# Ericonaldo/ILSwiss

Measured on AMD Instinct MI355X. Metric: env-steps/s + SAC grad-steps/s, Hopper-v2 4096 envs, higher is better.
Workload: dtype f32

## Files before the change

ilswiss_amd/csrc/host_common.h:

```cpp
#pragma once
#include <hip/hip_runtime.h>
#include <hip/hip_ext.h>

#include <cstdarg>
#include <cstdio>
#include <cstring>
#include <deque>
#include <string>
#include <utility>
#include <vector>

#include "../../include/ilsx.h"
#include "kernels.h"

void ilsx_set_err(const char* fmt, ...);

#define ILSX_FAIL(code, ...)   \
  do {                         \
    ilsx_set_err(__VA_ARGS__); \
    return (code);             \
  } while (0)

#define HIPCHK(expr)                                                                              \
  do {                                                                                            \
// ... 63 lines not shown
  std::vector<std::pair<void**, size_t>> items;
  size_t bytes = 0;
  template <class T> void add(T** p, size_t count) {
    bytes = (bytes + 255) & ~(size_t)255;
    items.push_back({(void**)p, bytes});
    bytes += count * sizeof(T);
  }
  int commit(ilsx_ctx* c, void** base) {
    int rc = ctx_alloc(c, bytes ? bytes : 256, base, true);
    if (rc != ILSX_OK) return rc;
    for (auto& it : items) *it.first = (char*)*base + it.second;
    return ILSX_OK;
  }
};
int ctx_free(ilsx_ctx* c, void* p);
int ctx_stage(ilsx_ctx* c, size_t bytes, void** out);

struct NetLayout {
  ilsx_mlp_cfg cfg;
  int KP = 0, NO = 0;
  int off_W[ILSX_MAX_HID], off_Wb[ILSX_MAX_HID], off_b[ILSX_MAX_HID], ld[ILSX_MAX_HID];
  int off_Wh = 0, off_bh = 0;
  size_t n_int = 0;
  size_t n_flat = 0;
  int hl[ILSX_MAX_HID] = {0, 0, 0};
  int out_of(int l) const { return hl[l] > 0 ? hl[l] : cfg.hidden; }
  int in_of(int l) const { return l == 0 ? cfg.in_dim : out_of(l - 1); }
};
int net_layout_build(const ilsx_mlp_cfg& cfg, NetLayout* L);
void net_flat_to_internal(const NetLayout& L, const float* flat, float* internal);
void net_internal_to_flat(const NetLayout& L, const float* internal, float* flat);
NetView net_view(const NetLayout& L, float* base);

struct ilsx_net {
  ilsx_ctx* ctx = nullptr;
  NetLayout lay;
  float* base = nullptr;
  bool owns = true;
  float* ws_out = nullptr;
  int ws_rows = 0;
  bool noise_policy = false;
  float noise = 0.f, noise_clip = 0.f, max_act = 1.f;
  bool out_linear = false;
  bool categorical = false;
};
int launch_categorical_act(ilsx_ctx* ctx, const float* z, int rows, int n, int deterministic, unsigned long long step, float* act, float* logp);

int net_upload_flat(ilsx_ctx* ctx, const NetLayout& L, float* dev_base, const float* src, size_t n, int src_is_device);
int net_download_flat(ilsx_ctx* ctx, const NetLayout& L, const float* dev_base, float* dst, size_t n, int dst_is_device);

int launch_fwd(ilsx_ctx* ctx, const FwdArgs& A, int H, int act, int KP, int cs = 1);
int launch_bwd_dx(ilsx_ctx* ctx, const BwdArgs& A, int H, int act, int cs = 1);
int launch_policy_finish(ilsx_ctx* ctx, const PolicyFinishArgs& P);
bool phase_fits(ilsx_ctx* ctx, int rows, int H, int cs, int ntasks);
struct PhaseConst {
  int slot = -1, device = 0;
  bool tried = false, valid_a = false, valid_c = false;
  unsigned long long key_a = 0, key_c = 0;
  PhaseAArgs a; PhaseCArgs c;
};
int phase_const_alloc(int device);
void phase_const_prepare(ilsx_ctx* ctx, PhaseConst* ct);
void phase_const_free(int device, int slot);
int launch_phase_a(ilsx_ctx* ctx, const PhaseAArgs& P, int H, int act, int KPmax, int cs, PhaseConst* ct = nullptr, unsigned long long key = 0, bool upload_only = false);
int launch_phase_c(ilsx_ctx* ctx, const PhaseCArgs& P, int H, int act, int KPmax, int cs, PhaseConst* ct = nullptr, unsigned long long key = 0, bool upload_only = false);
int device_cus(ilsx_ctx* ctx);
int grp_const_alloc(int device, bool fwd, int n, int* base);
void grp_const_free(int device, bool fwd, int base);
int grp_const_upload(ilsx_ctx* ctx, bool fwd, int base, const void* host_records, size_t count);
struct ilsx_sac;
int sac_staged_batch(ilsx_sac* s, int B, float** obs, float** act, float** rew, float** done, float** nobs);
int sac_step_staged(ilsx_sac* s, ilsx_sac_stats* stats);
int sac_dims(const ilsx_sac* s, int* o, int* a);
int sac_window_begin(ilsx_sac* s, int B);
int sac_window_step(ilsx_sac* s);
int sac_window_end(ilsx_sac* s, bool teardown = false);
#define ILSX_RETRY_WINDOW (-1000)
int sac_snapshot_take(ilsx_sac* s);
int sac_snapshot_restore(ilsx_sac* s);
bool sac_window_may_use_phase(ilsx_sac* s, int B);
int mlp2_split_factor(int n_hidden, int H);
int launch_bwd_dw(ilsx_ctx* ctx, const DwArgs& table, int rows, const AdamFuse* fuse = nullptr);
int dw_table_add(DwArgs* T, const float* A, int lda, int NA, const float* Bm, int ldb, int NB, float* dW, float* dWb, int ldw,
                 float* db, int mode, int rows = 0, int bias_rows = 0);
int launch_adam(ilsx_ctx* ctx, const AdamArgs& A);
int build_dw_jobs(const NetLayout& L, float* gbase, const float* xsave, float* const* hsave,
                  float* const* dsave, const float* dhead, DwArgs* table);

struct ilsx_replay {
  ilsx_ctx* ctx = nullptr;
  int64_t cap = 0;
  int o = 0, a = 0, rec = 0;
  float* data = nullptr;
  DevReplayState* dstate = nullptr;
  bool dstate_stale = false;
  uint64_t seed = 0;
  uint32_t rng_stream = 0;
  unsigned long long sample_ctr = 0;
  int64_t top = 0, size = 0, cur_start = 0;
  std::deque<std::pair<int64_t, int64_t>> trajs;
  std::vector<uint8_t> start_flag;
};
int replay_flush_state(ilsx_replay* rb);
int replay_advance_device_rows(ilsx_replay* rb, int n);
int replay_insert_paths(ilsx_replay* rb, const float* stage, int stage_len, const int* envs, const int* lens, const uint8_t* last_terminal,
                        int n_paths);
int replay_launch_sample(ilsx_replay* rb, int B, const int64_t* idx, const DevScalars* scal,
// ... 3 lines not shown
```

ilswiss_amd/csrc/ilsx_core.hip:

```cpp
#include <algorithm>
#include <cmath>
#include <cstdlib>
#include <random>

#define ILSX_KERNEL_IMPL 1
#include <mutex>
#include "host_common.h"

static thread_local std::string g_err = "";

void ilsx_set_err(const char* fmt, ...) {
  char buf[1024];
  va_list ap;
  va_start(ap, fmt);
  vsnprintf(buf, sizeof buf, fmt, ap);
  va_end(ap);
  g_err = buf;
}

static int kernels_init_once();
extern "C" int ilsx_abi_version(void) { return ILSX_ABI_VERSION; }
extern "C" const char* ilsx_last_error(void) { return g_err.c_str(); }

int ctx_alloc(ilsx_ctx* c, size_t bytes, void** out, bool zero) {
// ... 455 lines not shown
      if (act == ILSX_ACT_RELU) { if (gg == 2) L0_CALL(ACT_RELU, 2); else if (gg == 1) L0_CALL(ACT_RELU, 1); else L0_CALL(ACT_RELU, 0); }
      else { if (gg == 2) L0_CALL(ACT_TANH, 2); else if (gg == 1) L0_CALL(ACT_TANH, 1); else L0_CALL(ACT_TANH, 0); }
#undef L0_CALL
    } else if (H == 256 && cs == 4) {
#define FWD_GRP_CALL(HH, AA, CC) do { if (A.tasks && A.ctab && A.late) ILSX_LAUNCH(ps, (k_mlp2_fwd_split<HH, AA, CC, 3>), grid, block, lds, ctx->stream, A); \
        else if (A.tasks && A.ctab) ILSX_LAUNCH(ps, (k_mlp2_fwd_split<HH, AA, CC, 2>), grid, block, lds, ctx->stream, A); \
        else if (A.tasks) ILSX_LAUNCH(ps, (k_mlp2_fwd_split<HH, AA, CC, 1>), grid, block, lds, ctx->stream, A); \
        else ILSX_LAUNCH(ps, (k_mlp2_fwd_split<HH, AA, CC, 0>), grid, block, lds, ctx->stream, A); } while (0)
      if (act == ILSX_ACT_RELU) FWD_GRP_CALL(256, ACT_RELU, 4); else FWD_GRP_CALL(256, ACT_TANH, 4);
    } else if (H == 128 && cs == 2) {
      if (act == ILSX_ACT_RELU) FWD_GRP_CALL(128, ACT_RELU, 2); else FWD_GRP_CALL(128, ACT_TANH, 2);
#undef FWD_GRP_CALL
    } else {
      ILSX_FAIL(ILSX_ERR_UNSUPPORTED, "no column-split forward kernel for H=%d cs=%d", H, cs);
    }
    HIPCHK(hipGetLastError());
    return ILSX_OK;
  }
  const size_t lds = fwd_lds_bytes(H, KPmax);
  if (lds > 160 * 1024) ILSX_FAIL(ILSX_ERR_UNSUPPORTED, "forward tile needs %zu B of LDS (> 160 KiB)", lds);
  dim3 grid((A.rows + 15) / 16, A.ntasks), block(4 * H);
#define CALL_FWD(HH, AA) ILSX_LAUNCH(ps, (k_mlp_fwd<HH, AA>), grid, block, lds, ctx->stream, A)
  DISPATCH_H_ACT(H, act, CALL_FWD);
#undef CALL_FWD
  HIPCHK(hipGetLastError());
  return ILSX_OK;
}

int device_cus(ilsx_ctx* ctx) {
  static int n_cu = 0;
  if (!n_cu) {
    hipDeviceProp_t pr;
    n_cu = hipGetDeviceProperties(&pr, ctx->device) == hipSuccess ? pr.multiProcessorCount : 1;
  }
  return n_cu;
}
static size_t phase_lds_bytes(int H, int KP, int cs) { return std::max(fwd_split_lds_bytes(H, KP, cs), bwd_split_lds_bytes(H, cs)); }
void phase_wgs_per_cu(int H, int cs, int* occ_a, int* occ_c) {
  static int oa[2] = {-1, -1}, oc[2] = {-1, -1};
  const int i = H == 256 ? 0 : 1;
  if (oa[i] < 0) {
    int a = 0, c = 0;
    const size_t lds = phase_lds_bytes(H, 32, cs);
    hipError_t e1, e2;
    if (H == 256) { e1 = hipOccupancyMaxActiveBlocksPerMultiprocessor(&a, (const void*)k_sac_phase_a<256, ACT_RELU, 4>, 4 * H / cs, lds);
                    e2 = hipOccupancyMaxActiveBlocksPerMultiprocessor(&c, (const void*)k_sac_phase_c<256, ACT_RELU, 4>, 4 * H / cs, lds); }
    else { e1 = hipOccupancyMaxActiveBlocksPerMultiprocessor(&a, (const void*)k_sac_phase_a<128, ACT_RELU, 2>, 4 * H / cs, lds);
           e2 = hipOccupancyMaxActiveBlocksPerMultiprocessor(&c, (const void*)k_sac_phase_c<128, ACT_RELU, 2>, 4 * H / cs, lds); }
    oa[i] = e1 == hipSuccess ? std::max(a, 1) : 1;
    oc[i] = e2 == hipSuccess ? std::max(c, 1) : 1;
  }
  *occ_a = oa[i]; *occ_c = oc[i];
}
bool phase_fits(ilsx_ctx* ctx, int rows, int H, int cs, int ntasks) {
  const int n_cu = device_cus(ctx);
  if (!((H == 256 && cs == 4) || (H == 128 && cs == 2))) return false;
  const int tiles = (rows + 15) / 16, work = tiles * ntasks * cs;
  int occ_a = 1, occ_c = 1;
  phase_wgs_per_cu(H, cs, &occ_a, &occ_c);
  return tiles <= PHASE_MAX_TILES && work <= n_cu && work + 1 <= occ_a * n_cu && tiles * 3 * cs <= occ_c * n_cu;
}

static std::vector<bool> g_phase_slots[16];
static std::mutex g_phase_slots_mu;
int phase_const_alloc(int device) {
  static const bool off = []() { const char* e = getenv("ILSX_PHASE_CT"); return e && atoi(e) == 0; }();
  if (off || device < 0 || device >= 16) return -1;
  std::lock_guard<std::mutex> lock(g_phase_slots_mu);
  auto& u = g_phase_slots[device];
  if (u.empty()) u.assign(PHASE_CONST_SLOTS, false);
  for (int i = 0; i < PHASE_CONST_SLOTS; ++i) if (!u[i]) { u[i] = true; return i; }
  return -1;
}
void phase_const_free(int device, int slot) {
  if (device < 0 || device >= 16 || slot < 0 || slot >= PHASE_CONST_SLOTS) return;
  std::lock_guard<std::mutex> lock(g_phase_slots_mu);
  if (!g_phase_slots[device].empty()) g_phase_slots[device][slot] = false;
}
void phase_const_prepare(ilsx_ctx* ctx, PhaseConst* ct) {
  if (!ct || ct->tried) return;
  ct->tried = true;
  ct->device = ctx->device;
  ct->slot = phase_const_alloc(ctx->device);
  if (ct->slot >= 0) ctx->phase_slots.push_back(ct->slot);
}
template <class Blk>
static bool phase_const_ready(ilsx_ctx* ctx, PhaseConst* ct, const Blk& blk, unsigned long long key, Blk& held, bool& valid, unsigned long long& held_key,
                              const void* symbol) {
  phase_const_prepare(ctx, ct);
  if (!ct || ct->slot < 0 || blk.dbg || !key) return false;
  if (valid && held_key == key) return true;
  hipStreamCaptureStatus cap = hipStreamCaptureStatusNone;
  if (hipStreamIsCapturing(ctx->stream, &cap) != hipSuccess || cap != hipStreamCaptureStatusNone) return false;
  if (hipStreamSynchronize(ctx->stream) != hipSuccess) return false;
  valid = false;
  memcpy(&held, &blk, sizeof blk);
  if (hipMemcpyToSymbolAsync(symbol, &held, sizeof blk, (size_t)ct->slot * sizeof blk, hipMemcpyHostToDevice, ctx->stream) != hipSuccess ||
      hipStreamSynchronize(ctx->stream) != hipSuccess) { (void)hipGetLastError(); return false; }
  valid = true; held_key = key;
  return true;
}

int launch_phase_a(ilsx_ctx* ctx, const PhaseAArgs& P0, int H, int act, int KPmax, int cs, PhaseConst* ct, unsigned long long key, bool upload_only) {
  PhaseAArgs P = P0;
  P.f1.xs = P.f2.xs = P.b1.xs = 0; P.f1.rt = P.f2.rt = 1;
  P.f1.dbg = P.f2.dbg = nullptr; P.b1.dbg = nullptr;
  P.dbg = upload_only ? nullptr : ctx->dbg_next();
  if (P.b1.ga_parts < 1) P.b1.ga_parts = 1;
  const int tiles = (P.f1.rows + 15) / 16;
  dim3 grid((tiles + 7) & ~7, 5, cs), block(4 * H / cs);
  const size_t lds = phase_lds_bytes(H, KPmax, cs);
  const bool use_ct = ct && phase_const_ready(ctx, ct, P, key, ct->a, ct->valid_a, ct->key_a, HIP_SYMBOL(g_phase_a_tab));
  if (upload_only) return ILSX_OK;
  const int slot = use_ct ? ct->slot : 0;
  static const bool trace = getenv("ILSX_PHASE_CT_TRACE") != nullptr;
  if (trace) { hipStreamCaptureStatus cap = hipStreamCaptureStatusNone; hipStreamIsCapturing(ctx->stream, &cap);
               fprintf(stderr, "launch_phase_a: %s, slot %d, capturing %d\n", use_ct ? "constant table" : "kernel arguments", ct ? ct->slot : -9, (int)cap); }
  ProfScope ps(ctx, ILSX_K_SAC_PHASE_A);
#define PHASE_A(HH, AA, CC) do { if (use_ct) ILSX_LAUNCH(ps, (k_sac_phase_a<HH, AA, CC, true>), grid, block, lds, ctx->stream, P, slot); \
                                 else ILSX_LAUNCH(ps, (k_sac_phase_a<HH, AA, CC>), grid, block, lds, ctx->stream, P, slot); } while (0)
  if (H == 256 && act == ILSX_ACT_RELU) PHASE_A(256, ACT_RELU, 4);
  else if (H == 256) PHASE_A(256, ACT_TANH, 4);
  else if (act == ILSX_ACT_RELU) PHASE_A(128, ACT_RELU, 2);
  else PHASE_A(128, ACT_TANH, 2);
#undef PHASE_A
  HIPCHK(hipGetLastError());
  return ILSX_OK;
}

int launch_phase_c(ilsx_ctx* ctx, const PhaseCArgs& P0, int H, int act, int KPmax, int cs, PhaseConst* ct, unsigned long long key, bool upload_only) {
  PhaseCArgs P = P0;
  P.f3.xs = P.b2.xs = P.b3.xs = 0; P.f3.rt = 1;
  P.f3.dbg = nullptr; P.b2.dbg = P.b3.dbg = nullptr;
  P.dbg = upload_only ? nullptr : ctx->dbg_next();
  if (P.b2.ga_parts < 1) P.b2.ga_parts = 1;
  if (P.b3.ga_parts < 1) P.b3.ga_parts = 1;
  const int tiles = (P.f3.rows + 15) / 16;
  dim3 grid((tiles + 7) & ~7, 4, cs), block(4 * H / cs);
  const size_t lds = phase_lds_bytes(H, KPmax, cs);
  const bool use_ct = ct && phase_const_ready(ctx, ct, P, key, ct->c, ct->valid_c, ct->key_c, HIP_SYMBOL(g_phase_c_tab));
  if (upload_only) return ILSX_OK;
  const int slot = use_ct ? ct->slot : 0;
  ProfScope ps(ctx, ILSX_K_SAC_PHASE_C);
#define PHASE_C(HH, AA, CC) do { if (use_ct) ILSX_LAUNCH(ps, (k_sac_phase_c<HH, AA, CC, true>), grid, block, lds, ctx->stream, P, slot); \
                                 else ILSX_LAUNCH(ps, (k_sac_phase_c<HH, AA, CC>), grid, block, lds, ctx->stream, P, slot); } while (0)
  if (H == 256 && act == ILSX_ACT_RELU) PHASE_C(256, ACT_RELU, 4);
  else if (H == 256) PHASE_C(256, ACT_TANH, 4);
  else if (act == ILSX_ACT_RELU) PHASE_C(128, ACT_RELU, 2);
  else PHASE_C(128, ACT_TANH, 2);
#undef PHASE_C
  HIPCHK(hipGetLastError());
  return ILSX_OK;
}

int launch_bwd_dx(ilsx_ctx* ctx, const BwdArgs& A0, int H, int act, int cs) {
  if (A0.rows <= 0) return ILSX_OK;
  BwdArgs A = A0;
  A.dbg = ctx->dbg_next();
  if (A.ga_parts < 1) A.ga_parts = 1;
  ProfScope ps(ctx, ILSX_K_MLP_BWD_DX);
  if (cs > 1 && A.tasks && A.mt > 1) {
    if (!(H == 256 && cs == 4) || (A.mt != 2 && A.mt != 4)) ILSX_FAIL(ILSX_ERR_UNSUPPORTED, "macro-tile backward: H=%d cs=%d mt=%d", H, cs, A.mt);
    A.xs = 0; A.ctab = 0;
// ... 384 lines not shown
```

ilswiss_amd/csrc/ilsx_sac.hip:

```cpp
#include <cmath>
#include <cstdlib>

#include <algorithm>
#include "host_common.h"

enum { W_PI = 0, W_Q1 = 1, W_Q2 = 2, W_TQ1 = 3, W_TQ2 = 4 };

struct SacWs {
  float *s, *a, *r, *d, *s2, *eps1, *eps2;
  float *a2, *logp2, *q1, *q2, *tq1, *tq2;
  float *xq[2], *hq[2][ILSX_MAX_HID], *dq[2][ILSX_MAX_HID], *dhq[2];
  float *raw, *an, *logp, *epss, *q1n, *q2n, *ga[2];
  float *xp, *hp[ILSX_MAX_HID], *dp[ILSX_MAX_HID], *dhp;
  float* ppart;
  float* ppart2;
};

struct StatsArgs {
  PartVal q1, q2, tq1, tq2, q1n, q2n;
  const float *logp2, *r, *d, *logp, *raw;
  int B, a;
  float gamma, reward_scale, w_mu, w_std, target_entropy, inv_B;
  DevScalars* scal;
  float* alpha_grad_slot;
  int slot_given;
};

struct SacTailItem { StatsArgs S; int train_alpha; float lr, b1, b2, eps, qf_lr, policy_lr; };
struct SacLaunch {
  int kind;
  FwdArgs f; int KP; BwdArgs b; DwArgs d; AdamFuse F; SacTailItem t;
};
struct SacCollector { std::vector<SacLaunch> L; };

struct ilsx_sac {
  ilsx_ctx* ctx = nullptr;
  SacCollector* col = nullptr;
  ilsx_sac_cfg cfg;
  ilsx_net *pi = nullptr, *q1 = nullptr, *q2 = nullptr;
  NetLayout Lq, Lp;
  int o = 0, a = 0;
  size_t nq = 0, np = 0;
  void* slab = nullptr;
  float *P = nullptr, *G = nullptr, *M = nullptr, *V = nullptr;
  DevScalars* scal = nullptr;
  SacWs ws;
  DwArgs jobs_q, jobs_p;
  ilsx_replay* gather_rb = nullptr;
  bool fuse_now = false;
  int cs = 1;
  float* h0scr = nullptr;
  int B = 0;
  bool eps_explicit = false;
  float target_entropy = 0.f;
  uint32_t rng_stream = 0;
  hipGraphExec_t graph = nullptr;
  ilsx_replay* graph_rb = nullptr;
  int graph_B = 0;
  bool graph_defer = false, graph_phase = false;
  hipGraphExec_t seg_graph[3] = {nullptr, nullptr, nullptr};
  ilsx_replay* seg_rb = nullptr;
  int seg_B = 0;
  bool defer_tail = false;
  TailLite* tail_dev = nullptr;
  int tail_B = 0;
  ilsx_sac_stats stats_cache; bool stats_cached = false;
  bool tail_split = false;
  unsigned* phase_flags = nullptr;
  int* phase_err = nullptr;
  PhaseConst pct;
  bool phase_args_only = false;
  bool no_ct = false;
  bool phase_now = false;
  bool phase_broken = false;
  bool phase_last = false;
  bool debug_break = false;
  int phase_fallbacks = 0;
  float* vote = nullptr;
  bool snap_valid = false;
  void* snap = nullptr;
  size_t snap_bytes = 0;
  float* base(int which) const {
    switch (which) {
      case W_Q1: return P;
      case W_Q2: return P + nq;
      case W_PI: return P + 2 * nq;
      case W_TQ1: return P + 2 * nq + np;
      default: return P + 3 * nq + np;
    }
  }
  PartVal pv(const float* p) const { return PartVal{p, cs, cfg.max_batch}; }
  float* gbase(int which) const { return which == W_Q1 ? G : which == W_Q2 ? G + nq : G + 2 * nq; }
  size_t trainable_off(int which) const { return which == W_Q1 ? 0 : which == W_Q2 ? nq : 2 * nq; }
};


__device__ __forceinline__ void sac_alpha_grad_dev(const StatsArgs& S) {
  __shared__ float sh2[4];
  float lpe = 0.f;
  for (int r = threadIdx.x; r < S.B; r += 256) lpe += S.logp[r] + S.target_entropy;
  lpe = block256_sum(lpe, sh2);
  if (threadIdx.x == 0) {
    S.scal->alpha_used = S.scal->alpha;
    S.scal->log_alpha_used = S.scal->log_alpha;
    if (!S.slot_given) {
      S.alpha_grad_slot[0] = -lpe * S.inv_B;
      S.alpha_grad_slot[1] = 0.f; S.alpha_grad_slot[2] = 0.f; S.alpha_grad_slot[3] = 0.f;
    }
  }
}

__device__ __forceinline__ void sac_stats_dev(const StatsArgs& S) {
// ... 244 lines not shown
  } else {
    t.eps = eps; t.action = action; t.logp = logp;
    if (save) { t.out = w.raw; t.eps_save = w.epss; }
  }
}
static void sac_policy_fin(ilsx_sac* s, FwdArgs& A, const float* eps, uint32_t stream, bool save, float* action, float* logp,
                           const float* part) {
  if (s->cs == 1) return;
  const SacWs& w = s->ws;
  PolicyFinishArgs& P = A.fin;
  memset(&P, 0, sizeof P);
  P.part = part; P.cs = s->cs; P.part_stride = s->cfg.max_batch; P.rows = s->B; P.a = s->a;
  P.head = HEAD_TANH_SAMPLE; P.rng_stream = stream; P.seed = s->ctx->seed; P.scal = s->scal;
  P.eps = eps; P.action = action; P.logp = logp;
  if (save) { P.raw = w.raw; P.eps_save = w.epss; }
  A.fin_on = 1;
}
static void sac_q_task(ilsx_sac* s, FwdTask& q, int which, const float* obs, const float* act, float* out, bool save_x,
                       bool save_h, int i) {
  const SacWs& w = s->ws;
  q.net = net_view(s->Lq, s->base(which));
  q.x0 = obs; q.d0 = s->o; q.s0 = s->o; q.x1 = act; q.d1 = s->a; q.s1 = s->a;
  if (save_x) q.xsave = w.xq[i];
  if (save_h) for (int l = 0; l < s->Lq.cfg.n_hidden; ++l) q.hsave[l] = w.hq[i][l];
  q.head = HEAD_RAW;
  if (s->cs > 1) q.part = out; else q.out = out;
}

static int sac_fwd(ilsx_sac* s, const FwdArgs& A0, int H, int act, int KP, int cs) {
  FwdArgs A = A0;
  if (s->h0scr) {
    A.l0_split = 1;
    for (int t = 0; t < A.ntasks; ++t)
      if (!A.t[t].hsave[0]) A.t[t].hsave[0] = s->h0scr + (size_t)t * s->cfg.max_batch * H;
  }
  if (!s->col) return launch_fwd(s->ctx, A, H, act, KP, cs);
  SacLaunch l; memset(&l, 0, sizeof l); l.kind = 0; l.f = A; l.KP = KP;
  s->col->L.push_back(l);
  return ILSX_OK;
}
static int sac_bwd(ilsx_sac* s, const BwdArgs& A, int H, int act, int cs) {
  if (!s->col) return launch_bwd_dx(s->ctx, A, H, act, cs);
  SacLaunch l; memset(&l, 0, sizeof l); l.kind = 1; l.b = A;
  s->col->L.push_back(l);
  return ILSX_OK;
}
static int sac_dw(ilsx_sac* s, const DwArgs& table, int rows, const AdamFuse* F) {
  if (!s->col) return launch_bwd_dw(s->ctx, table, rows, F);
  SacLaunch l; memset(&l, 0, sizeof l); l.kind = 2; l.d = table; l.F = *F;
  s->col->L.push_back(l);
  return ILSX_OK;
}

static unsigned long long sac_phase_key(const ilsx_sac* s) {
  unsigned long long k = 1469598103934665603ull;
  auto mix = [&k](unsigned long long v) { k = (k ^ v) * 1099511628211ull; };
  const ilsx_replay* rb = s->gather_rb;
  mix((unsigned long long)(uintptr_t)rb); mix(rb ? (unsigned long long)(uintptr_t)rb->data : 0); mix(rb ? (unsigned long long)(uintptr_t)rb->dstate : 0);
  mix(rb ? (unsigned long long)rb->rec : 0); mix(rb ? (unsigned long long)rb->seed : 0); mix(rb ? (unsigned long long)rb->rng_stream : 0);
  mix((unsigned long long)s->B); mix(s->defer_tail ? 1 : 0); mix(s->eps_explicit ? 1 : 0); mix(s->fuse_now ? 1 : 0); mix((unsigned long long)s->cs);
  mix((unsigned long long)(uintptr_t)s->tail_dev); mix((unsigned long long)(uintptr_t)s->slab);
  return k ? k : 1;
}

static int sac_critic_backward(ilsx_sac* s) {
  const SacWs& w = s->ws;
  const int B = s->B, H = s->Lq.cfg.hidden, act = s->Lq.cfg.act, cs = s->cs;
  const float* eps1 = s->eps_explicit ? w.eps1 : nullptr;
  const float* eps2 = s->eps_explicit ? w.eps2 : nullptr;
  PhaseAArgs PA;
  if (s->phase_now) memset(&PA, 0, sizeof PA);
  {
    FwdArgs A;
    memset(&A, 0, sizeof A);
    A.rows = B; A.ntasks = 4; A.seed = s->ctx->seed; A.scal = s->scal; A.part_stride = s->cfg.max_batch;
    sac_policy_task(s, A.t[0], w.s2, eps1, s->rng_stream, false, w.a2, w.logp2, w.ppart);
    sac_policy_task(s, A.t[3], w.s, eps2, s->rng_stream + 1, true, w.an, w.logp, w.ppart2);
    sac_q_task(s, A.t[1], W_Q1, w.s, w.a, w.q1, true, true, 0);
    sac_q_task(s, A.t[2], W_Q2, w.s, w.a, w.q2, true, true, 1);
    if (s->gather_rb && cs > 1) {
      ilsx_replay* rb = s->gather_rb;
      GatherSpec& G = A.gather;
      G.records = rb->data; G.st = rb->dstate; G.rec = rb->rec; G.seed = rb->seed; G.stream = rb->rng_stream;
      G.o = s->o; G.adim = s->a; G.on = 1;
      G.s = w.s; G.a = w.a; G.r = w.r; G.d = w.d; G.s2 = w.s2;
      A.t[0].g0_off = s->o + s->a + 2; A.t[0].publish = 2;
      A.t[1].g0_off = 0; A.t[1].g1_off = s->o; A.t[1].publish = 1;
      A.t[2].g0_off = 0; A.t[2].g1_off = s->o; A.t[2].publish = 0;
      A.t[3].g0_off = 0; A.t[3].publish = 0;
    }
    if (s->defer_tail) { A.tail = s->tail_dev; A.tail_mode = 1; A.tail_n = 1; }
    if (s->phase_now) PA.f1 = A;
    else ILSX_TRY(sac_fwd(s, A, H, act, std::max(s->Lq.KP, s->Lp.KP), cs));
  }
  {
    FwdArgs A;
    memset(&A, 0, sizeof A);
    A.rows = B; A.ntasks = 2; A.seed = s->ctx->seed; A.scal = s->scal; A.part_stride = s->cfg.max_batch;
    sac_q_task(s, A.t[0], W_TQ1, w.s2, w.a2, w.tq1, false, false, 0);
    sac_q_task(s, A.t[1], W_TQ2, w.s2, w.a2, w.tq2, false, false, 1);
    sac_policy_fin(s, A, eps1, s->rng_stream, false, w.a2, w.logp2, w.ppart);
    if (s->defer_tail) { A.tail = s->tail_dev; A.tail_mode = 2; A.tail_n = 1; }
    if (s->phase_now) {
      A.fin.use_gather_step = 1;
      A.tail_mode = 0;
      PA.f2 = A;
    } else {
      ILSX_TRY(sac_fwd(s, A, H, act, s->Lq.KP, cs));
    }
  }
  {
    BwdArgs A;
    memset(&A, 0, sizeof A);
    A.rows = B; A.ntasks = 2; A.inv_B = sac_inv_B(s);
    A.gamma = s->cfg.discount; A.reward_scale = s->cfg.reward_scale; A.scal = s->scal;
    A.part_stride = s->cfg.max_batch;
    for (int i = 0; i < 2; ++i) {
      BwdTask& t = A.t[i];
      t.net = net_view(s->Lq, s->base(i == 0 ? W_Q1 : W_Q2));
      for (int l = 0; l < s->Lq.cfg.n_hidden; ++l) { t.hsave[l] = w.hq[i][l]; t.dsave[l] = w.dq[i][l]; }
      t.dhead = w.dhq[i];
      t.loss = LOSS_SAC_CRITIC;
      t.q = s->pv(i == 0 ? w.q1 : w.q2); t.tq1 = s->pv(w.tq1); t.tq2 = s->pv(w.tq2);
      t.logp_next = w.logp2; t.rew = w.r; t.done = w.d;
    }
    if (s->phase_now) {
      PA.b1 = A; PA.flags = s->phase_flags; PA.err = s->phase_err;
      {
        FwdArgs Fz;
        memset(&Fz, 0, sizeof Fz);
        sac_policy_fin(s, Fz, eps2, s->rng_stream + 1, true, w.an, w.logp, w.ppart2);
        PA.fin_pi = Fz.fin; PA.fin_pi.use_gather_step = 1; PA.fin_pi_on = 1;
      }
      ILSX_TRY(launch_phase_a(s->ctx, PA, H, act, std::max(s->Lq.KP, s->Lp.KP), cs, s->no_ct ? nullptr : &s->pct, sac_phase_key(s), s->phase_args_only));
      if (s->phase_args_only) return ILSX_OK;
    } else {
      ILSX_TRY(sac_bwd(s, A, H, act, cs));
    }
  }
  AdamFuse F;
  memset(&F, 0, sizeof F);
  if (s->fuse_now) {
    F.on = 1; F.Gbase = s->G; F.P = s->P; F.M = s->M; F.V = s->V; F.T = s->base(W_TQ1);
    F.b1 = s->cfg.beta_1; F.b2 = 0.999f; F.eps = 1e-8f; F.tau = s->cfg.soft_target_tau;
    F.step_size = &s->scal->adam_q_step; F.bc2_sqrt = &s->scal->adam_q_bc2s;
    if (s->phase_now) F.T = nullptr;
  }
  return sac_dw(s, s->jobs_q, B, &F);
}

static int sac_critic_update(ilsx_sac* s) {
  if (s->fuse_now) return ILSX_OK;
  AdamArgs A;
  A.p = s->P; A.g = s->G; A.m = s->M; A.v = s->V; A.tgt = s->base(W_TQ1);
  A.n = (int)(2 * s->nq);
  A.b1 = s->cfg.beta_1; A.b2 = 0.999f; A.eps = 1e-8f; A.tau = s->cfg.soft_target_tau;
  A.step_size = &s->scal->adam_q_step; A.bc2_sqrt = &s->scal->adam_q_bc2s;
  return launch_adam(s->ctx, A);
}

static StatsArgs sac_stats_args(ilsx_sac* s);
static int sac_actor_backward(ilsx_sac* s) {
  const SacWs& w = s->ws;
  const int B = s->B, H = s->Lq.cfg.hidden, act = s->Lq.cfg.act, cs = s->cs;
  const float* eps2 = s->eps_explicit ? w.eps2 : nullptr;
  PhaseCArgs PC;
  if (s->phase_now) memset(&PC, 0, sizeof PC);
  {
    FwdArgs A;
    memset(&A, 0, sizeof A);
    A.rows = B; A.ntasks = 2; A.seed = s->ctx->seed; A.scal = s->scal; A.part_stride = s->cfg.max_batch;
    sac_q_task(s, A.t[0], W_Q1, w.s, w.an, w.q1n, false, true, 0);
    sac_q_task(s, A.t[1], W_Q2, w.s, w.an, w.q2n, false, true, 1);
    if (!s->phase_now) sac_policy_fin(s, A, eps2, s->rng_stream + 1, true, w.an, w.logp, w.ppart2);
    if (s->phase_now) { A.tail = s->tail_dev; PC.f3 = A; }
    else ILSX_TRY(sac_fwd(s, A, H, act, s->Lq.KP, cs));
  }
  {
    BwdArgs A;
    memset(&A, 0, sizeof A);
// ... 455 lines not shown
extern "C" int ilsx_sac_phase_state(ilsx_sac* s, int* fallbacks, int* disabled, int* last_window_on_phase, int* wgs_per_cu_a, int* wgs_per_cu_c) {
  if (!s) ILSX_FAIL(ILSX_ERR_ARG, "ilsx_sac_phase_state: NULL agent");
  if (fallbacks) *fallbacks = s->phase_fallbacks;
  if (disabled) *disabled = s->phase_broken ? 1 : 0;
  if (last_window_on_phase) *last_window_on_phase = s->phase_last ? 1 : 0;
  int oa = 0, oc = 0;
  if (s->cs > 1 && (s->Lq.cfg.hidden == 256 || s->Lq.cfg.hidden == 128)) phase_wgs_per_cu(s->Lq.cfg.hidden, s->cs, &oa, &oc);
  if (wgs_per_cu_a) *wgs_per_cu_a = oa;
  if (wgs_per_cu_c) *wgs_per_cu_c = oc;
  return ILSX_OK;
}
extern "C" int ilsx_sac_debug_break_phase(ilsx_sac* s) {
  if (!s) ILSX_FAIL(ILSX_ERR_ARG, "ilsx_sac_debug_break_phase: NULL agent");
  static const int one = 1;
  HIPCHK(hipSetDevice(s->ctx->device));
  HIPCHK(hipMemcpyAsync(s->phase_err, &one, sizeof one, hipMemcpyHostToDevice, s->ctx->stream));
  s->debug_break = true;
  return ILSX_OK;
}
static int sac_train_from_replay_once(ilsx_sac* s, ilsx_replay* rb, int n_steps, int B, ilsx_sac_stats* stats) {
  if (!s || !rb || n_steps < 0) ILSX_FAIL(ILSX_ERR_ARG, "ilsx_sac_train_from_replay: bad argument");
  if (B < 1 || B > s->cfg.max_batch) ILSX_FAIL(ILSX_ERR_ARG, "batch %d not in 1..max_batch=%d", B, s->cfg.max_batch);
  if (rb->o != s->o || rb->a != s->a) ILSX_FAIL(ILSX_ERR_ARG, "replay dims (%d,%d) != agent dims (%d,%d)", rb->o, rb->a, s->o, s->a);
  if (rb->size < 1) ILSX_FAIL(ILSX_ERR_STATE, "replay buffer is empty");
  ILSX_TRY(sac_check_world(s, "ilsx_sac_train_from_replay"));
  HIPCHK(hipSetDevice(s->ctx->device));
  ILSX_TRY(replay_flush_state(rb));
  hipStream_t st = s->ctx->stream;
  s->B = B;
  s->eps_explicit = false;
  static const bool split_graph = getenv("ILSX_SPLIT_GRAPH") != nullptr;
  static const bool no_graph_env = getenv("ILSX_NO_GRAPH") != nullptr;
  const bool no_graph = no_graph_env || (sac_is_split(s) && !split_graph);
  if (n_steps == 0) return stats ? sac_read_stats(s, stats) : ILSX_OK;
  ILSX_TRY(sac_defer_begin(s, B));
  struct DeferGuard { ilsx_sac* s; ~DeferGuard() { s->defer_tail = false; } } guard{s};
  const bool deferred = s->defer_tail;
  if (deferred && sac_window_may_use_phase(s, B)) ILSX_TRY(sac_snapshot_take(s));
  static const bool segments = []() { const char* e = getenv("ILSX_SPLIT_SEGMENTS"); return e && atoi(e) != 0; }();
  if (sac_is_split(s) && !split_graph && !no_graph_env && segments && !s->ctx->prof_on) {
    for (int i = 0; i < n_steps; ++i) {
      if (stats && i == n_steps - 1) ILSX_TRY(sac_request_stats(s));
      ILSX_TRY(sac_split_segments_step(s, rb, B));
    }
  } else if (no_graph || s->ctx->prof_on) {
    for (int i = 0; i < n_steps; ++i) {
      if (stats && i == n_steps - 1) ILSX_TRY(sac_request_stats(s));
      const int rc = sac_sample_and_step(s, rb, B);
      if (rc != ILSX_OK) return rc;
    }
  } else {
    const bool phase = sac_phase_ok(s, B);
    s->phase_last = phase;
    static const bool no_reprime = getenv("ILSX_PHASE_CT_NO_REPRIME") != nullptr;
    const bool rebuild = !s->graph || s->graph_rb != rb || s->graph_B != B || s->graph_defer != s->defer_tail || s->graph_phase != phase;
    if (phase && (rebuild || !no_reprime)) ILSX_TRY(sac_phase_const_prime(s, rb));
    if (!s->graph || s->graph_rb != rb || s->graph_B != B || s->graph_defer != s->defer_tail || s->graph_phase != phase) {
      if (s->graph) { hipGraphExecDestroy(s->graph); s->graph = nullptr; }
      hipGraph_t g = nullptr;
      HIPCHK(hipStreamBeginCapture(st, hipStreamCaptureModeThreadLocal));
      int rc = sac_sample_and_step(s, rb, B);
      hipError_t e = hipStreamEndCapture(st, &g);
      if (rc != ILSX_OK) { if (g) hipGraphDestroy(g); return rc; }
      if (e != hipSuccess) ILSX_FAIL(ILSX_ERR_HIP, "hipStreamEndCapture failed: %s", hipGetErrorString(e));
      e = hipGraphInstantiate(&s->graph, g, nullptr, nullptr, 0);
      hipGraphDestroy(g);
      if (e != hipSuccess) { s->graph = nullptr; ILSX_FAIL(ILSX_ERR_HIP, "hipGraphInstantiate failed: %s", hipGetErrorString(e)); }
      s->graph_rb = rb; s->graph_B = B; s->graph_defer = s->defer_tail; s->graph_phase = phase;
    }
    for (int i = 0; i < n_steps; ++i) {
      if (stats && i == n_steps - 1) ILSX_TRY(sac_request_stats(s));
      HIPCHK(hipGraphLaunch(s->graph, st));
    }
  }
  s->defer_tail = false;
  ILSX_TRY(sac_flush_tail(s, deferred));
  ILSX_TRY(sac_phase_check(s, B, deferred, "ilsx_sac_train_from_replay"));
  if (stats) return sac_read_stats(s, stats);
  return ILSX_OK;
}

static const NetLayout* sac_layout(const ilsx_sac* s, int which) { return which == W_PI ? &s->Lp : &s->Lq; }

extern "C" int ilsx_sac_get_params(ilsx_sac* s, int which, float* dst, size_t n, int dst_is_device) {
  if (!s || !dst || which < 0 || which > 4) ILSX_FAIL(ILSX_ERR_ARG, "ilsx_sac_get_params: bad argument");
  HIPCHK(hipSetDevice(s->ctx->device));
  return net_download_flat(s->ctx, *sac_layout(s, which), s->base(which), dst, n, dst_is_device);
}
extern "C" int ilsx_sac_set_params(ilsx_sac* s, int which, const float* src, size_t n, int src_is_device) {
  if (!s || !src || which < 0 || which > 4) ILSX_FAIL(ILSX_ERR_ARG, "ilsx_sac_set_params: bad argument");
  HIPCHK(hipSetDevice(s->ctx->device));
  return net_upload_flat(s->ctx, *sac_layout(s, which), s->base(which), src, n, src_is_device);
}
extern "C" int ilsx_sac_get_grads(ilsx_sac* s, int which, float* dst, size_t n, int dst_is_device) {
  if (!s || !dst || which < 0 || which > 2) ILSX_FAIL(ILSX_ERR_ARG, "ilsx_sac_get_grads: bad argument");
  HIPCHK(hipSetDevice(s->ctx->device));
  return net_download_flat(s->ctx, *sac_layout(s, which), s->gbase(which), dst, n, dst_is_device);
}
extern "C" int ilsx_sac_grads_ptr(ilsx_sac* s, int segment, float** dev_ptr, size_t* n) {
  if (!s || !dev_ptr || !n || segment < 0 || segment > 1) ILSX_FAIL(ILSX_ERR_ARG, "ilsx_sac_grads_ptr: bad argument");
  if (segment == 0) { *dev_ptr = s->G; *n = 2 * s->nq; }
  else { *dev_ptr = s->G + 2 * s->nq; *n = s->np + 4; }
  return ILSX_OK;
}
extern "C" int ilsx_sac_get_log_alpha(ilsx_sac* s, double* out) {
  if (!s || !out) ILSX_FAIL(ILSX_ERR_ARG, "NULL argument");
  HIPCHK(hipSetDevice(s->ctx->device));
  DevScalars h;
  HIPCHK(hipMemcpyAsync(&h, s->scal, sizeof h, hipMemcpyDeviceToHost, s->ctx->stream));
  HIPCHK(hipStreamSynchronize(s->ctx->stream));
  *out = h.log_alpha;
  return ILSX_OK;
}
extern "C" int ilsx_sac_set_log_alpha(ilsx_sac* s, double v) {
  if (!s) ILSX_FAIL(ILSX_ERR_ARG, "NULL argument");
  HIPCHK(hipSetDevice(s->ctx->device));
  DevScalars h;
  HIPCHK(hipMemcpyAsync(&h, s->scal, sizeof h, hipMemcpyDeviceToHost, s->ctx->stream));
  HIPCHK(hipStreamSynchronize(s->ctx->stream));
  h.log_alpha = v;
  h.alpha = (float)std::exp(v);
// ... 434 lines not shown
```

ilswiss_amd/csrc/kernels.h:

```cpp
#pragma once
#include <hip/hip_runtime.h>
#include <stdint.h>

typedef float f32x4 __attribute__((ext_vector_type(4)));

#define ILSX_LDS_PAD 4
#ifndef ILSX_LATE_WAVES
#define ILSX_LATE_WAVES 4
#endif
#ifndef ILSX_MT_WAVES
#define ILSX_MT_WAVES 2
#endif
#define ILSX_MAX_HID 3
#define ILSX_MAX_NO 64

enum { HEAD_RAW = 0, HEAD_TANH_SAMPLE = 1, HEAD_TANH_DET = 2, HEAD_TANH_LOGP_OF_ACT = 3,
       HEAD_GAUSS_SAMPLE = 4, HEAD_GAUSS_LOGP_OF_ACT = 5,
       HEAD_DET_TANH_NOISE = 6,
       HEAD_DET_LIN_NOISE = 7 };
enum { LOSS_GIVEN = 0, LOSS_SAC_CRITIC = 1, LOSS_SAC_ACTORQ = 2, LOSS_SAC_POLICY = 3, LOSS_MSE = 4, LOSS_PPO_POLICY = 5,
       LOSS_TD_CRITIC = 6, LOSS_SACV_VALUE = 7, LOSS_CONST = 8, LOSS_TD3_POLICY = 9, LOSS_BC_MLE = 10, LOSS_BC_MSE = 11 };
enum { ACT_RELU = 0, ACT_TANH = 1 };

#define LOG_SIG_MIN (-20.0f)
// ... 855 lines not shown
      const float ls = fminf(fmaxf(lsr, LOG_SIG_MIN), LOG_SIG_MAX);
      const float sd = expf(ls);
      float e = 0.f, z, act;
      if (P.head == HEAD_TANH_DET) {
        z = mu; act = tanhf(mu);
      } else if (P.head == HEAD_TANH_LOGP_OF_ACT) {
        act = P.act_in[(size_t)gr * a + j];
        z = 0.5f * (logf(1.0f + act + TANH_EPS) - logf(1.0f - act + TANH_EPS));
      } else {
        e = P.eps ? P.eps[(size_t)gr * a + j] : z4[jj];
        z = e * sd + mu;
        act = tanhf(z);
      }
      const float dm = mu - z;
      lp_quad += dm * dm / expf(2.0f * ls);
      lp_ls += ls;
      lp_jac += logf(1.0f - act * act + TANH_EPS);
      if (P.action) P.action[(size_t)gr * a + j] = act;
      if (P.eps_save) P.eps_save[(size_t)gr * a + j] = e;
    }
  }
  if (P.logp) P.logp[gr] = -0.5f * lp_quad - (lp_ls + HALF_LOG_2PI) - lp_jac;
}

template <int H, int ACT, int CS, int GRP, int MT = 1>
__global__ __launch_bounds__(4 * H / CS, (MT > 1 ? ILSX_MT_WAVES : GRP == 3 ? ILSX_LATE_WAVES : 1)) void k_mlp2_bwd_split(const BwdArgs A) {
  extern __shared__ __attribute__((aligned(16))) float smem[];
  static_assert(MT == 1 || GRP, "macro tiles are a grouped-launch shape");
  int sw_bx = 0, sw_task = 0, sw_cs = 0;
  if constexpr (GRP && MT > 1) {
    if (!grp_swizzle(A.swz, CS, blockIdx.x, &sw_bx, &sw_task, &sw_cs)) return;
  }
  const int ty = (GRP && MT > 1) ? sw_task : (int)blockIdx.y;
  BwdTask Tg;
  if (GRP == 1) Tg = A.tasks[ty];
  const BwdTask& T = GRP >= 2 ? g_bwd_tab[A.ctab - 1 + ty] : GRP == 1 ? Tg : A.t[ty];
  constexpr bool XCH = false;
  const int bx = (GRP && MT > 1) ? sw_bx : (int)blockIdx.x, cs = (GRP && MT > 1) ? sw_cs : (int)blockIdx.z;
#define XCH_HOOK_ACT
#define XCH_HOOK_HEAD
#include "bwd_split_tile.inc"
#undef XCH_HOOK_ACT
#undef XCH_HOOK_HEAD
}
#endif

#define PHASE_MAX_TILES 64
#define PHASE_TAIL_FLAG (3 * PHASE_MAX_TILES)
#define PHASE_NFLAGS (3 * PHASE_MAX_TILES + 1)
#define PHASE_MASK_WORD(t) ((PHASE_NFLAGS + (t)) * 32)
#define PHASE_FLAG_WORDS ((PHASE_NFLAGS + PHASE_MAX_TILES) * 32)
struct PhaseAArgs {
  FwdArgs f1, f2; BwdArgs b1; unsigned* flags; int* err; unsigned long long* dbg;
  PolicyFinishArgs fin_pi; int fin_pi_on, pad;
};
struct PhaseCArgs {
  FwdArgs f3; BwdArgs b2, b3; unsigned* flags; int* err; unsigned long long* dbg;
  float* polyak_T; const float* polyak_P; int polyak_n; float polyak_tau;
  float* aslot; const float* aslot_logp; int aslot_B; float aslot_te, aslot_invB;
};

static_assert(sizeof(PhaseAArgs) <= 4096 && sizeof(PhaseCArgs) <= 4096, "phase-kernel descriptors travel in the kernel-argument segment (4 KB)");
#define PHASE_CONST_SLOTS 64
#ifdef ILSX_KERNEL_IMPL
__constant__ PhaseAArgs g_phase_a_tab[PHASE_CONST_SLOTS];
__constant__ PhaseCArgs g_phase_c_tab[PHASE_CONST_SLOTS];
#endif

#ifdef ILSX_KERNEL_IMPL
__device__ __forceinline__ void xch_arrive(unsigned* flag) {
  asm volatile("s_waitcnt vmcnt(0)" ::: "memory");
  __syncthreads();
  if (threadIdx.x == 0) __hip_atomic_fetch_add(flag, 1u, __ATOMIC_RELAXED, __HIP_MEMORY_SCOPE_AGENT);
}
#define PHASE_FLAG_DEAD 0x40000000u
__device__ __forceinline__ void xch_wait(const unsigned* flag, unsigned target, int* err) {
  if (threadIdx.x == 0) {
    int spins = 0;
    while (__hip_atomic_load(flag, __ATOMIC_RELAXED, __HIP_MEMORY_SCOPE_AGENT) < target) {
      __builtin_amdgcn_s_sleep(2);
      if (++spins > (1 << 16)) { __hip_atomic_store(err, 1, __ATOMIC_RELAXED, __HIP_MEMORY_SCOPE_AGENT); break; }
    }
  }
  __syncthreads();
  asm volatile("buffer_inv sc0" ::: "memory");
}
__device__ __forceinline__ unsigned xcc_id() {
  unsigned v;
  asm volatile("s_getreg_b32 %0, hwreg(HW_REG_XCC_ID)" : "=s"(v));
  return v & 15u;
}
__device__ __forceinline__ void xch_mark_xcd(unsigned* mask) {
  if (threadIdx.x == 0) __hip_atomic_fetch_or(mask, 1u << xcc_id(), __ATOMIC_RELAXED, __HIP_MEMORY_SCOPE_AGENT);
}

__device__ __forceinline__ void policy_fin_tile(const PolicyFinishArgs& P, int r0, int rows, float* lp3, int nth) {
  const int a = P.a, NOp = 2 * a, tid = threadIdx.x;
  const unsigned long long fstep = P.scal ? (P.use_gather_step ? P.scal->gather_step : P.scal->step) : P.step_host;
  for (int e = tid; e < 16 * a; e += nth) {
    const int row = e / a, j = e - row * a, gr = r0 + row;
    float c0 = 0.0f, c1 = 0.0f, c2 = 0.0f;
    if (gr < rows) {
      float pm[4], pl[4];
#pragma unroll
      for (int c = 0; c < 4; ++c) {
        const size_t at = ((size_t)(c < P.cs ? c : 0) * P.part_stride + gr) * NOp + j;
        pm[c] = P.part[at];
        pl[c] = P.part[at + a];
      }
      float mu = 0.f, lsr = 0.f;
#pragma unroll
      for (int c = 0; c < 4; ++c) { mu += c < P.cs ? pm[c] : 0.0f; lsr += c < P.cs ? pl[c] : 0.0f; }
      float ep;
      if (P.eps) {
        ep = P.eps[(size_t)gr * a + j];
      } else {
        float z4[4];
        philox_normal4(P.seed, fstep, P.rng_stream, gr, j >> 2, z4);
        const int q = j & 3;
        ep = q == 0 ? z4[0] : q == 1 ? z4[1] : q == 2 ? z4[2] : z4[3];
      }
      const float ls = fminf(fmaxf(lsr, LOG_SIG_MIN), LOG_SIG_MAX);
      const float sd = expf(ls);
      const float z = ep * sd + mu;
      const float act = tanhf(z);
      const float dm = mu - z;
      c0 = dm * dm / expf(2.0f * ls); c1 = ls; c2 = logf(1.0f - act * act + TANH_EPS);
      if (P.raw) { P.raw[(size_t)gr * NOp + j] = mu; P.raw[(size_t)gr * NOp + a + j] = lsr; }
      if (P.action) P.action[(size_t)gr * a + j] = act;
      if (P.eps_save) P.eps_save[(size_t)gr * a + j] = ep;
    }
    lp3[(row * 32 + j) * 3 + 0] = c0; lp3[(row * 32 + j) * 3 + 1] = c1; lp3[(row * 32 + j) * 3 + 2] = c2;
  }
  lds_barrier();
  if (P.logp && tid < 16 && r0 + tid < rows) {
    float q = 0.f, l = 0.f, jc = 0.f;
    for (int j = 0; j < a; ++j) { q += lp3[(tid * 32 + j) * 3]; l += lp3[(tid * 32 + j) * 3 + 1]; jc += lp3[(tid * 32 + j) * 3 + 2]; }
    P.logp[r0 + tid] = -0.5f * q - (l + HALF_LOG_2PI) - jc;
  }
  lds_barrier();
}

template <int H, int ACT, int CS, bool CT = false>
__global__ __launch_bounds__(4 * H / CS) void k_sac_phase_a(const PhaseAArgs Pk, int slot) {
  const PhaseAArgs& P = CT ? g_phase_a_tab[slot] : Pk;
  constexpr int GRP = 0; constexpr bool XCH = true;
  constexpr int PH = 0, MT = 1;
  extern __shared__ __attribute__((aligned(16))) float smem[];
  const FwdGroup* GP = nullptr;
  const int bx = blockIdx.x, cs = blockIdx.z, y = blockIdx.y;
  unsigned* tflag = P.flags + PHASE_TAIL_FLAG * 32;
  if (y == 4) {
    if (bx == 0 && cs == 0) {
      const TailLite& TL = P.f1.tail[0];
      tail_lite_run(TL, smem);
      if (threadIdx.x == 0) {
        __hip_atomic_store(&TL.scal->alpha, TL.scal->alpha, __ATOMIC_RELAXED, __HIP_MEMORY_SCOPE_AGENT);
        asm volatile("s_waitcnt vmcnt(0)" ::: "memory");
        __hip_atomic_store(tflag, 1u, __ATOMIC_RELAXED, __HIP_MEMORY_SCOPE_AGENT);
      }
    }
    return;
  }
  if (bx * 16 >= P.f1.rows) return;
  unsigned* f1 = P.flags + (3 * bx) * 32;
  unsigned* f2 = P.flags + (3 * bx + 1) * 32;
  ILSX_STAMP(P.dbg, 0);
#if defined(ILSX_STAMPS) && defined(ILSX_STAMPS_FINE)
  if (P.dbg && threadIdx.x == 0 && (y == 1 || y == 2)) P.dbg[(size_t)ILSX_WG_LINEAR * ILSX_TRACE_SLOTS + 5] = clock64();
#endif
  xch_mark_xcd(P.flags + PHASE_MASK_WORD(bx));
  {
    const FwdArgs& A = P.f1;
    const FwdTask& T = A.t[y];
    const bool first_task = y == 0;
#define XCH_HOOK_STAGE
#define XCH_HOOK_FIN
#include "fwd_split_tile.inc"
#undef XCH_HOOK_STAGE
#undef XCH_HOOK_FIN
  }
  ILSX_STAMP(P.dbg, 1);
  unsigned* f0 = P.flags + (3 * bx + 2) * 32;
  if (y == 0) {
    asm volatile("s_waitcnt vmcnt(0)" ::: "memory");
    __syncthreads();
    if (threadIdx.x == 0) {
      __hip_atomic_fetch_add(f0, 1u, __ATOMIC_RELAXED, __HIP_MEMORY_SCOPE_AGENT);
      __hip_atomic_fetch_add(f1, 1u, __ATOMIC_RELAXED, __HIP_MEMORY_SCOPE_AGENT);
    }
  } else {
    xch_arrive(f1);
  }
  ILSX_STAMP(P.dbg, 2);
  if (y == 0 || y == 3) {
    {
      const FwdArgs& A = P.f2;
      const FwdTask& T = A.t[y == 0 ? 0 : 1];
      const bool first_task = y == 0;
#define XCH_HOOK_STAGE ILSX_STAMP_SYNC(P.dbg, 7); xch_wait(f0, CS, P.err); ILSX_STAMP(P.dbg, 3);
#define XCH_HOOK_FIN
#define XCH_FINE_DBG P.dbg
#include "fwd_split_tile.inc"
#undef XCH_FINE_DBG
#undef XCH_HOOK_STAGE
#undef XCH_HOOK_FIN
    }
    ILSX_STAMP(P.dbg, 4);
    xch_arrive(f2);
    ILSX_STAMP(P.dbg, 5);
  } else {
    xch_wait(f1, 4 * CS, P.err);
    if (P.fin_pi_on && y == 1 && cs == 0) {
      xch_wait(tflag, 1u, P.err);
      policy_fin_tile(P.fin_pi, bx * 16, P.f1.rows, smem, 4 * H / CS);
    }
    {
      const BwdArgs& A = P.b1;
      const BwdTask& T = A.t[y - 1];
#define XCH_HOOK_ACT
#define XCH_HOOK_HEAD xch_wait(f2, 2 * CS, P.err); xch_wait(tflag, 1u, P.err); ILSX_STAMP(P.dbg, 3);
#include "bwd_split_tile.inc"
#undef XCH_HOOK_ACT
#undef XCH_HOOK_HEAD
    }
    ILSX_STAMP(P.dbg, 4);
#if defined(ILSX_STAMPS) && defined(ILSX_STAMPS_FINE)
    if (P.dbg && threadIdx.x == 0) P.dbg[(size_t)ILSX_WG_LINEAR * ILSX_TRACE_SLOTS + 6] = clock64();
#endif
  }
}

template <int H, int ACT, int CS, bool CT = false>
__global__ __launch_bounds__(4 * H / CS) void k_sac_phase_c(const PhaseCArgs Pk, int slot) {
  const PhaseCArgs& P = CT ? g_phase_c_tab[slot] : Pk;
  constexpr int GRP = 0; constexpr bool XCH = true;
  constexpr int PH = 0, MT = 1;
  extern __shared__ __attribute__((aligned(16))) float smem[];
  const FwdGroup* GP = nullptr;
  const int bx = blockIdx.x, cs = blockIdx.z, y = blockIdx.y;
  if (y == 3) {
    if (bx == 0 && cs == 0 && threadIdx.x == 0) P.f3.tail[0].scal->gather_step += 1;
    if (P.aslot && bx == 1 && cs == 0) alpha_slot_run(P.aslot_logp, P.aslot_B, P.aslot_te, P.aslot_invB, P.aslot, smem);
    const float tau = P.polyak_tau;
    for (int i = ((int)(cs * gridDim.x + bx) * (int)blockDim.x + (int)threadIdx.x) * 4; i < P.polyak_n; i += (int)(gridDim.x * gridDim.z * blockDim.x) * 4) {
      const float4 p = *reinterpret_cast<const float4*>(P.polyak_P + i);
      float4 t = *reinterpret_cast<const float4*>(P.polyak_T + i);
      t.x = t.x * (1.0f - tau) + p.x * tau; t.y = t.y * (1.0f - tau) + p.y * tau;
      t.z = t.z * (1.0f - tau) + p.z * tau; t.w = t.w * (1.0f - tau) + p.w * tau;
      *reinterpret_cast<float4*>(P.polyak_T + i) = t;
    }
    return;
// ... 739 lines not shown
```

Before: 17340.

## Run phase-A second forward on dedicated workgroups instead of reusing first-pass ones

Adds an own-rows mode to the fused phase-A kernel: the grid grows from 5 to 7 y-slices, and two new workgroup slices run the f2 forward tasks. The y==0 and y==3 workgroups now return right after finishing their f1 task instead of going on to run f2. This lets the f2 work start as soon as its flag is set, rather than waiting behind the f1 work queued on the same workgroup. It costs extra workgroups, which must still fit co-resident for the spin-wait scheme, so the fit check now counts them. It is on by default when the occupancy check passes, can be disabled with an env var, and a CU-id debug stamp is added.

Result: faster. 17820 (median of 6 runs) (+2.8%).

```diff
diff --git a/ilswiss_amd/csrc/host_common.h b/ilswiss_amd/csrc/host_common.h
--- a/ilswiss_amd/csrc/host_common.h
+++ b/ilswiss_amd/csrc/host_common.h
@@ -139,7 +139,8 @@
 int launch_fwd(ilsx_ctx* ctx, const FwdArgs& A, int H, int act, int KP, int cs = 1);
 int launch_bwd_dx(ilsx_ctx* ctx, const BwdArgs& A, int H, int act, int cs = 1);
 int launch_policy_finish(ilsx_ctx* ctx, const PolicyFinishArgs& P);
-bool phase_fits(ilsx_ctx* ctx, int rows, int H, int cs, int ntasks);
+bool phase_fits(ilsx_ctx* ctx, int rows, int H, int cs, int ntasks, bool own_rows = false);
+bool phase_own_rows(ilsx_ctx* ctx, int rows, int H, int cs, int ntasks);
 struct PhaseConst {
   int slot = -1, device = 0;
   bool tried = false, valid_a = false, valid_c = false;
diff --git a/ilswiss_amd/csrc/ilsx_core.hip b/ilswiss_amd/csrc/ilsx_core.hip
--- a/ilswiss_amd/csrc/ilsx_core.hip
+++ b/ilswiss_amd/csrc/ilsx_core.hip
@@ -531,13 +531,18 @@
   }
   *occ_a = oa[i]; *occ_c = oc[i];
 }
-bool phase_fits(ilsx_ctx* ctx, int rows, int H, int cs, int ntasks) {
+bool phase_fits(ilsx_ctx* ctx, int rows, int H, int cs, int ntasks, bool own_rows) {
   const int n_cu = device_cus(ctx);
   if (!((H == 256 && cs == 4) || (H == 128 && cs == 2))) return false;
   const int tiles = (rows + 15) / 16, work = tiles * ntasks * cs;
   int occ_a = 1, occ_c = 1;
   phase_wgs_per_cu(H, cs, &occ_a, &occ_c);
-  return tiles <= PHASE_MAX_TILES && work <= n_cu && work + 1 <= occ_a * n_cu && tiles * 3 * cs <= occ_c * n_cu;
+  const int work_a = work + (own_rows ? tiles * 2 * cs : 0);
+  return tiles <= PHASE_MAX_TILES && work <= n_cu && work_a + 1 <= occ_a * n_cu && tiles * 3 * cs <= occ_c * n_cu;
+}
+bool phase_own_rows(ilsx_ctx* ctx, int rows, int H, int cs, int ntasks) {
+  const char* e = getenv("ILSX_PHASE_OWN_ROWS");
+  return !(e && atoi(e) == 0) && phase_fits(ctx, rows, H, cs, ntasks, true);
 }
 
 static std::vector<bool> g_phase_slots[16];
@@ -587,7 +592,7 @@
   P.dbg = upload_only ? nullptr : ctx->dbg_next();
   if (P.b1.ga_parts < 1) P.b1.ga_parts = 1;
   const int tiles = (P.f1.rows + 15) / 16;
-  dim3 grid((tiles + 7) & ~7, 5, cs), block(4 * H / cs);
+  dim3 grid((tiles + 7) & ~7, P.own_rows ? 7 : 5, cs), block(4 * H / cs);
   const size_t lds = phase_lds_bytes(H, KPmax, cs);
   const bool use_ct = ct && phase_const_ready(ctx, ct, P, key, ct->a, ct->valid_a, ct->key_a, HIP_SYMBOL(g_phase_a_tab));
   if (upload_only) return ILSX_OK;
diff --git a/ilswiss_amd/csrc/ilsx_sac.hip b/ilswiss_amd/csrc/ilsx_sac.hip
--- a/ilswiss_amd/csrc/ilsx_sac.hip
+++ b/ilswiss_amd/csrc/ilsx_sac.hip
@@ -57,7 +57,7 @@
   hipGraphExec_t graph = nullptr;
   ilsx_replay* graph_rb = nullptr;
   int graph_B = 0;
-  bool graph_defer = false, graph_phase = false;
+  bool graph_defer = false, graph_phase = false, graph_own = false;
   hipGraphExec_t seg_graph[3] = {nullptr, nullptr, nullptr};
   ilsx_replay* seg_rb = nullptr;
   int seg_B = 0;
@@ -408,6 +408,7 @@
   return ILSX_OK;
 }
 
+static bool sac_own_rows(const ilsx_sac* s) { return phase_own_rows(s->ctx, s->B, s->Lq.cfg.hidden, s->cs, 4); }
 static unsigned long long sac_phase_key(const ilsx_sac* s) {
   unsigned long long k = 1469598103934665603ull;
   auto mix = [&k](unsigned long long v) { k = (k ^ v) * 1099511628211ull; };
@@ -416,6 +417,7 @@
   mix(rb ? (unsigned long long)rb->rec : 0); mix(rb ? (unsigned long long)rb->seed : 0); mix(rb ? (unsigned long long)rb->rng_stream : 0);
   mix((unsigned long long)s->B); mix(s->defer_tail ? 1 : 0); mix(s->eps_explicit ? 1 : 0); mix(s->fuse_now ? 1 : 0); mix((unsigned long long)s->cs);
   mix((unsigned long long)(uintptr_t)s->tail_dev); mix((unsigned long long)(uintptr_t)s->slab);
+  mix(sac_own_rows(s) ? 1 : 0);
   return k ? k : 1;
 }
 
@@ -482,6 +484,7 @@
     }
     if (s->phase_now) {
       PA.b1 = A; PA.flags = s->phase_flags; PA.err = s->phase_err;
+      PA.own_rows = sac_own_rows(s) ? 1 : 0;
       {
         FwdArgs Fz;
         memset(&Fz, 0, sizeof Fz);
@@ -1043,10 +1046,11 @@
   } else {
     const bool phase = sac_phase_ok(s, B);
     s->phase_last = phase;
+    const bool own = phase && sac_own_rows(s);
     static const bool no_reprime = getenv("ILSX_PHASE_CT_NO_REPRIME") != nullptr;
-    const bool rebuild = !s->graph || s->graph_rb != rb || s->graph_B != B || s->graph_defer != s->defer_tail || s->graph_phase != phase;
+    const bool rebuild = !s->graph || s->graph_rb != rb || s->graph_B != B || s->graph_defer != s->defer_tail || s->graph_phase != phase || s->graph_own != own;
     if (phase && (rebuild || !no_reprime)) ILSX_TRY(sac_phase_const_prime(s, rb));
-    if (!s->graph || s->graph_rb != rb || s->graph_B != B || s->graph_defer != s->defer_tail || s->graph_phase != phase) {
+    if (rebuild) {
       if (s->graph) { hipGraphExecDestroy(s->graph); s->graph = nullptr; }
       hipGraph_t g = nullptr;
       HIPCHK(hipStreamBeginCapture(st, hipStreamCaptureModeThreadLocal));
@@ -1057,7 +1061,7 @@
       e = hipGraphInstantiate(&s->graph, g, nullptr, nullptr, 0);
       hipGraphDestroy(g);
       if (e != hipSuccess) { s->graph = nullptr; ILSX_FAIL(ILSX_ERR_HIP, "hipGraphInstantiate failed: %s", hipGetErrorString(e)); }
-      s->graph_rb = rb; s->graph_B = B; s->graph_defer = s->defer_tail; s->graph_phase = phase;
+      s->graph_rb = rb; s->graph_B = B; s->graph_defer = s->defer_tail; s->graph_phase = phase; s->graph_own = own;
     }
     for (int i = 0; i < n_steps; ++i) {
       if (stats && i == n_steps - 1) ILSX_TRY(sac_request_stats(s));
diff --git a/ilswiss_amd/csrc/kernels.h b/ilswiss_amd/csrc/kernels.h
--- a/ilswiss_amd/csrc/kernels.h
+++ b/ilswiss_amd/csrc/kernels.h
@@ -931,7 +931,8 @@
 #define PHASE_FLAG_WORDS ((PHASE_NFLAGS + PHASE_MAX_TILES) * 32)
 struct PhaseAArgs {
   FwdArgs f1, f2; BwdArgs b1; unsigned* flags; int* err; unsigned long long* dbg;
-  PolicyFinishArgs fin_pi; int fin_pi_on, pad;
+  PolicyFinishArgs fin_pi; int fin_pi_on;
+  int own_rows;
 };
 struct PhaseCArgs {
   FwdArgs f3; BwdArgs b2, b3; unsigned* flags; int* err; unsigned long long* dbg;
@@ -968,6 +969,11 @@
   unsigned v;
   asm volatile("s_getreg_b32 %0, hwreg(HW_REG_XCC_ID)" : "=s"(v));
   return v & 15u;
+}
+__device__ __forceinline__ unsigned cu_key() {
+  unsigned v;
+  asm volatile("s_getreg_b32 %0, hwreg(HW_REG_HW_ID)" : "=s"(v));
+  return (xcc_id() << 8) | ((v >> 8) & 255u);
 }
 __device__ __forceinline__ void xch_mark_xcd(unsigned* mask) {
   if (threadIdx.x == 0) __hip_atomic_fetch_or(mask, 1u << xcc_id(), __ATOMIC_RELAXED, __HIP_MEMORY_SCOPE_AGENT);
@@ -1044,39 +1050,47 @@
   if (bx * 16 >= P.f1.rows) return;
   unsigned* f1 = P.flags + (3 * bx) * 32;
   unsigned* f2 = P.flags + (3 * bx + 1) * 32;
+  unsigned* f0 = P.flags + (3 * bx + 2) * 32;
+  const bool own = y >= 5;
   ILSX_STAMP(P.dbg, 0);
 #if defined(ILSX_STAMPS) && defined(ILSX_STAMPS_FINE)
   if (P.dbg && threadIdx.x == 0 && (y == 1 || y == 2)) P.dbg[(size_t)ILSX_WG_LINEAR * ILSX_TRACE_SLOTS + 5] = clock64();
 #endif
   xch_mark_xcd(P.flags + PHASE_MASK_WORD(bx));
-  {
-    const FwdArgs& A = P.f1;
-    const FwdTask& T = A.t[y];
-    const bool first_task = y == 0;
+#if defined(ILSX_STAMPS) && !defined(ILSX_STAMPS_FINE)
+  if (P.dbg && threadIdx.x == 0 && ILSX_WG_LINEAR < ILSX_TRACE_MAXWG) P.dbg[(size_t)ILSX_WG_LINEAR * ILSX_TRACE_SLOTS + 7] = 0x10000u | cu_key();
+#endif
+  if (!own) {
+    {
+      const FwdArgs& A = P.f1;
+      const FwdTask& T = A.t[y];
+      const bool first_task = y == 0;
 #define XCH_HOOK_STAGE
 #define XCH_HOOK_FIN
 #include "fwd_split_tile.inc"
 #undef XCH_HOOK_STAGE
 #undef XCH_HOOK_FIN
-  }
-  ILSX_STAMP(P.dbg, 1);
-  unsigned* f0 = P.flags + (3 * bx + 2) * 32;
-  if (y == 0) {
-    asm volatile("s_waitcnt vmcnt(0)" ::: "memory");
-    __syncthreads();
-    if (threadIdx.x == 0) {
-      __hip_atomic_fetch_add(f0, 1u, __ATOMIC_RELAXED, __HIP_MEMORY_SCOPE_AGENT);
-      __hip_atomic_fetch_add(f1, 1u, __ATOMIC_RELAXED, __HIP_MEMORY_SCOPE_AGENT);
-    }
-  } else {
-    xch_arrive(f1);
-  }
-  ILSX_STAMP(P.dbg, 2);
-  if (y == 0 || y == 3) {
+    }
+    ILSX_STAMP(P.dbg, 1);
+    if (y == 0) {
+      asm volatile("s_waitcnt vmcnt(0)" ::: "memory");
+      __syncthreads();
+      if (threadIdx.x == 0) {
+        __hip_atomic_fetch_add(f0, 1u, __ATOMIC_RELAXED, __HIP_MEMORY_SCOPE_AGENT);
+        __hip_atomic_fetch_add(f1, 1u, __ATOMIC_RELAXED, __HIP_MEMORY_SCOPE_AGENT);
+      }
+    } else {
+      xch_arrive(f1);
+    }
+    ILSX_STAMP(P.dbg, 2);
+    if (P.own_rows && (y == 0 || y == 3)) return;
+  }
+  if (y == 0 || y == 3 || own) {
     {
       const FwdArgs& A = P.f2;
-      const FwdTask& T = A.t[y == 0 ? 0 : 1];
-      const bool first_task = y == 0;
+      const int tq = own ? y - 5 : (y == 0 ? 0 : 1);
+      const FwdTask& T = A.t[tq];
+      const bool first_task = tq == 0;
 #define XCH_HOOK_STAGE ILSX_STAMP_SYNC(P.dbg, 7); xch_wait(f0, CS, P.err); ILSX_STAMP(P.dbg, 3);
 #define XCH_HOOK_FIN
 #define XCH_FINE_DBG P.dbg
```
